# iden3/wasmsnark

Measured on AMD Instinct MI355X. Metric: BN128 Groth16 prove ms @ 2^20 constraints, lower is better.
Workload: dtype u256 (Montgomery; 9x29-bit limbs, v_mad_u64_u32); 1 GPU; BN128 full Groth16 prove, synthetic 2^20-constraint R1CS (1-3 non-zeros per column of A and B, every variable present), key and witness resident in HBM, r and s injected; parallelism=1 GPU, no collective, lanes=2, device=AMD Radeon Graphics gfx950:sramecc+:xnack- CUs=256 device=0

## Files before the change

wasmsnark_amd/csrc/msm.hip:

```cpp
#include <string.h>

#include <algorithm>
#include <chrono>

#include "internal.h"
namespace wsnark {

#ifndef WS_ACC_WAVES
#define WS_ACC_WAVES 3
#endif
#ifndef WS_ACC_WAVES_G2
#define WS_ACC_WAVES_G2 2
#endif
#ifndef WS_G2_PREFETCH
#define WS_G2_PREFETCH 0
#endif
#ifndef WS_G1_PREFETCH
#define WS_G1_PREFETCH 1
#endif
#ifndef WS_MADD_WIDE
#define WS_MADD_WIDE 1
#endif
static const uint32_t CHUNK = 8;
#ifndef WS_TAIL_L2_DEFAULT
#define WS_TAIL_L2_DEFAULT 4
#endif

struct MsmScratch {
    DevBuf vals_out, entries, hot, hot_sums;
    DevBuf bstart, bend, buckets, counters, tasks, multi, partials;
    DevBuf chunkS, chunkA, sums, points_conv;
    DevBuf hot_done;
    DevBuf tree_half, tree_done;
};

static const uint32_t PRESORT_MAX_BINS = 4096;
static const uint32_t CNT_HIST = 16, CNT_CURSOR = 16 + 512, CNT_BINS = 2048;

template <class Fn>
__device__ __forceinline__ void for_each_digit(const Fe& raw, uint32_t c, uint32_t Wall, uint32_t w_off, uint32_t w_stride, Fn f) {
    const Fe s = Fr::reduce_full(raw);
    const uint32_t NB = 1u << (c - 1);
    uint32_t carry = 0, k = 0;
    for (uint32_t w = 0; w < Wall; w++) {
        const uint32_t bit = w * c;
        const uint32_t limb = bit >> 6, off = bit & 63;
        uint64_t v = limb < 4 ? (s.l[limb] >> off) : 0;
        if (off + c > 64 && limb + 1 < 4) v |= s.l[limb + 1] << (64 - off);
        uint32_t d = (uint32_t)(v & ((1u << c) - 1)) + carry;
        uint32_t neg = 0;
        if (d > NB) { d = (1u << c) - d; neg = 1; carry = 1; } else carry = 0;
        if (w >= w_off && (w - w_off) % w_stride == 0) {
            if (d) f(k, d, neg);
            k++;
        }
    }
}

struct PresortArgs {
    const Fe* scalars;
    uint32_t n, c, Wall, w_off, w_stride;
    uint32_t i0, i_end;
    uint32_t lo_bits, HB, nbins;
    uint32_t tile;
    uint32_t idx_bits;
    const uint8_t* mask;
    uint32_t flat;
};
__device__ __forceinline__ uint32_t presort_bin(const PresortArgs& A, uint32_t k, uint32_t d) {
    return (A.flat ? 0u : k * A.HB) + ((d - 1) >> A.lo_bits);
}

template <class E> struct PresortEntry;
template <> struct PresortEntry<uint64_t> {
    static __device__ __forceinline__ uint64_t make(uint32_t i, uint32_t neg, uint32_t lo, uint32_t) {
        return ((uint64_t)lo << 32) | (uint64_t)(i | (neg << 31));
    }
    static __device__ __forceinline__ uint32_t lo(uint64_t e, uint32_t) { return (uint32_t)(e >> 32); }
    static __device__ __forceinline__ uint32_t val(uint64_t e, uint32_t) { return (uint32_t)e; }
};
template <> struct PresortEntry<uint32_t> {
    static __device__ __forceinline__ uint32_t make(uint32_t i, uint32_t neg, uint32_t lo, uint32_t ib) {
        return i | (neg << ib) | (lo << (ib + 1));
    }
    static __device__ __forceinline__ uint32_t lo(uint32_t e, uint32_t ib) { return e >> (ib + 1); }
    static __device__ __forceinline__ uint32_t val(uint32_t e, uint32_t ib) {
        return (e & ((1u << ib) - 1)) | (((e >> ib) & 1u) << 31);
    }
};

// ... 199 lines not shown
    if (act == 0) return 0;
    const uint32_t lane = threadIdx.x & 63;
    const int first = __ffsll(act) - 1;
    const uint32_t k0 = __shfl(key, first);
    const unsigned long long same = __ballot(active && key == k0);
    uint32_t r = 0;
    if (same == act) {
        uint32_t base = 0;
        if (lane == (uint32_t)first) base = atomicAdd(&counters[k0], (uint32_t)__popcll(act));
        base = __shfl(base, first);
        r = base + (uint32_t)__popcll(act & ((1ull << lane) - 1));
    } else if (active) {
        r = atomicAdd(&counters[key], 1u);
    }
    return r;
}

__device__ __forceinline__ uint32_t presort_bins_bounds(uint32_t bin, uint32_t s, uint32_t lo_bits, uint32_t lmax, uint32_t* sub, uint32_t* off,
                                                        uint32_t* wsum, uint32_t* lhist, uint32_t* __restrict__ bstart,
                                                        uint32_t* __restrict__ bend, uint32_t* __restrict__ hist) {
    const uint32_t SUB = 1u << lo_bits;
    const uint32_t per = (SUB + blockDim.x - 1) / blockDim.x, t0 = threadIdx.x * per;
    uint32_t mine = 0, bin_total;
    for (uint32_t t = t0; t < t0 + per && t < SUB; t++) mine += sub[t];
    uint32_t run = s + block_exclusive_scan(mine, wsum, &bin_total);
    for (uint32_t t = t0; t < t0 + per && t < SUB; t++) {
        const uint32_t cnt = sub[t];
        const uint32_t bucket = (bin << lo_bits) + t;
        off[t] = run;
        bstart[bucket] = run;
        bend[bucket] = run + cnt;
        run += cnt;
        sub[t] = 0;
        if (cnt) {
            const uint32_t nt = (cnt + lmax - 1) / lmax, rem = cnt - (nt - 1) * lmax;
            if (nt > 1) atomicAdd(&lhist[255], nt - 1);
            atomicAdd(&lhist[len_key(rem, lmax)], 1u);
        }
    }
    __syncthreads();
    for (uint32_t t = threadIdx.x; t < 256; t += blockDim.x)
        if (lhist[t]) atomicAdd(&hist[t], lhist[t]);
    return bin_total;
}

static const uint32_t PRESORT_BINS_CAP = 4096;
static_assert(PRESORT_BINS_CAP < 0xFFFFu, "ranks are kept in 16 bits, 0xFFFF marks a masked entry");
static_assert(PRESORT_BINS_CAP * (4 + 4 + 2) + (2u << PRESORT_MAX_LO) * 4 + (17 + 256) * 4 <= PRESORT_LDS_BYTES / 3, "staged presort_bins: three workgroups per CU");
template <class E, bool STAGED>
__global__ __launch_bounds__(1024) void presort_bins(const E* __restrict__ entries, const uint32_t* __restrict__ bin_start,
                                                       uint32_t lo_bits, uint32_t idx_bits, uint32_t* __restrict__ vals_out,
                                                       uint32_t* __restrict__ bstart, uint32_t* __restrict__ bend,
                                                       uint32_t lmax, uint32_t* __restrict__ hist,
                                                       const uint8_t* __restrict__ mask, uint32_t mask_mod) {
    __shared__ uint32_t sub[1u << PRESORT_MAX_LO];
    __shared__ uint32_t off[1u << PRESORT_MAX_LO];
    __shared__ uint32_t wsum[17];
    __shared__ uint32_t lhist[256];
    const uint32_t bin = blockIdx.x, SUB = 1u << lo_bits;
    const uint32_t s = bin_start[bin], e = bin_start[bin + 1];
    for (uint32_t t = threadIdx.x; t < SUB; t += blockDim.x) sub[t] = 0;
    for (uint32_t t = threadIdx.x; t < 256; t += blockDim.x) lhist[t] = 0;
    __syncthreads();
    const uint32_t stride = 4 * blockDim.x;
    const uint32_t iters = (e - s + stride - 1) / stride;
    const bool staged = STAGED && e - s <= PRESORT_BINS_CAP;
    (void)staged;
    if constexpr (STAGED) {
        __shared__ uint32_t st_in[PRESORT_BINS_CAP];
        __shared__ uint32_t st_out[PRESORT_BINS_CAP];
        __shared__ uint16_t st_rank[PRESORT_BINS_CAP];
        if (staged) {
            for (uint32_t it = 0; it < iters; it++) {
                const uint32_t i = s + threadIdx.x + it * stride;
                E v[4];
#pragma unroll
                for (uint32_t u = 0; u < 4; u++) {
                    const uint32_t j = i + u * blockDim.x;
                    v[u] = j < e ? entries[j] : (E)0;
                }
#pragma unroll
                for (uint32_t u = 0; u < 4; u++) {
                    const uint32_t j = i + u * blockDim.x;
                    bool active = j < e;
                    if (mask && active) {
                        const uint32_t idx = PresortEntry<E>::val(v[u], idx_bits) & 0x7FFFFFFFu;
                        active = mask[mask_mod ? idx % mask_mod : idx] != 0;
                    }
                    const uint32_t r = wave_rank_add(sub, PresortEntry<E>::lo(v[u], idx_bits), active);
                    if (j < e) {
                        st_in[j - s] = (uint32_t)v[u];
                        st_rank[j - s] = active ? (uint16_t)r : (uint16_t)0xFFFFu;
                    }
                }
            }
            __syncthreads();
            const uint32_t kept = presort_bins_bounds(bin, s, lo_bits, lmax, sub, off, wsum, lhist, bstart, bend, hist);
            for (uint32_t j = threadIdx.x; j < e - s; j += blockDim.x) {
                const uint32_t r = st_rank[j];
                if (r != 0xFFFFu) {
                    const E v = (E)st_in[j];
                    st_out[off[PresortEntry<E>::lo(v, idx_bits)] - s + r] = PresortEntry<E>::val(v, idx_bits);
                }
            }
            __syncthreads();
            for (uint32_t j = threadIdx.x; j < kept; j += blockDim.x) vals_out[s + j] = st_out[j];
            return;
        }
    }
    for (uint32_t it = 0; it < iters; it++) {
        const uint32_t i = s + threadIdx.x + it * stride;
        E v[4];
#pragma unroll
// ... 162 lines not shown
        first[threadIdx.x] += v;
        __syncthreads();
    }
    if (blockIdx.x == 0 && threadIdx.x == 0) counters[3] = first[0];
    const uint32_t excl = threadIdx.x + 1 < 256 ? first[threadIdx.x + 1] : 0;
    __syncthreads();
    first[threadIdx.x] = excl;
    __syncthreads();
    const uint32_t b = blockIdx.x * blockDim.x + threadIdx.x;
    uint32_t cnt = 0, s = 0, nt = 0, rem = 0, krem = 0, r255 = 0, rrem = 0;
    if (b < nbuckets) {
        s = bstart[b];
        cnt = bend[b] - s;
        if (cnt) {
            nt = (cnt + lmax - 1) / lmax;
            rem = cnt - (nt - 1) * lmax;
            krem = len_key(rem, lmax);
            if (nt > 1) r255 = atomicAdd(&lcnt[255], nt - 1);
            rrem = atomicAdd(&lcnt[krem], 1u);
        }
    }
    __syncthreads();
    lbase[threadIdx.x] = lcnt[threadIdx.x] ? first[threadIdx.x] + atomicAdd(&cursor[threadIdx.x], lcnt[threadIdx.x]) : 0;
    __syncthreads();
    if (!cnt) return;
    if (nt == 1) {
        tasks[lbase[krem] + rrem] = Task{b, s, rem};
    } else {
        const uint32_t pbase = atomicAdd(&counters[0], nt);
        if (nt >= hot_min) {
            const uint32_t nsl = (nt + HOT_SLICE - 1) / HOT_SLICE;
            hot[atomicAdd(&counters[4], 1u)] = HotBucket{b, pbase, nt, lbase[255] + r255, lbase[krem] + rrem, s, rem,
                                                         atomicAdd(&counters[5], nsl)};
            return;
        }
        multi[atomicAdd(&counters[1], 1u)] = MultiBucket{b, pbase, nt};
        for (uint32_t k = 0; k + 1 < nt; k++) tasks[lbase[255] + r255 + k] = Task{PARTIAL_FLAG | (pbase + k), s + k * lmax, lmax};
        tasks[lbase[krem] + rrem] = Task{PARTIAL_FLAG | (pbase + nt - 1), s + (nt - 1) * lmax, rem};
    }
}

__global__ __launch_bounds__(256) void msm_plan_emit_hot(const HotBucket* __restrict__ hot, const uint32_t* __restrict__ counters,
                                                           uint32_t lmax, Task* __restrict__ tasks) {
    const uint32_t nhot = counters[4];
    for (uint32_t hb = blockIdx.x; hb < nhot; hb += gridDim.x) {
        const HotBucket h = hot[hb];
        for (uint32_t k = threadIdx.x; k + 1 < h.ntasks; k += blockDim.x)
            tasks[h.task_base + k] = Task{PARTIAL_FLAG | (h.first_partial + k), h.start + k * lmax, lmax};
        if (threadIdx.x == 0)
            tasks[h.rem_index] = Task{PARTIAL_FLAG | (h.first_partial + h.ntasks - 1), h.start + (h.ntasks - 1) * lmax, h.rem};
    }
}

template <class C>
struct AccSets {
    const typename C::AffP* points[4];
    const uint32_t* vals[4];
    const Task* tasks[4];
    const uint32_t* counters[4];
    const MultiBucket* multi[4];
    const HotBucket* hot[4];
    typename C::PtP* buckets[4];
    typename C::PtP* partials[4];
    typename C::PtP* hot_sums[4];
    uint32_t* hot_done[4];
};

template <class C>
__global__ __launch_bounds__(256, (sizeof(typename C::PtP) > 128 ? WS_ACC_WAVES_G2 : WS_ACC_WAVES)) void msm_accumulate(AccSets<C> as) {
    const typename C::AffP* __restrict__ points = as.points[blockIdx.y];
    const uint32_t* __restrict__ vals = as.vals[blockIdx.y];
    const Task* __restrict__ tasks = as.tasks[blockIdx.y];
    const uint32_t* __restrict__ counters = as.counters[blockIdx.y];
    typename C::PtP* __restrict__ buckets = as.buckets[blockIdx.y];
    typename C::PtP* __restrict__ partials = as.partials[blockIdx.y];
    const uint32_t t = blockIdx.x * blockDim.x + threadIdx.x;
    if (t >= counters[3]) return;
    const Task k = tasks[t];
    const typename C::PtP acc = C::pack_pt(accumulate_range<C>(points, vals, k.start, k.len));
    if (k.dst & PARTIAL_FLAG) partials[k.dst & ~PARTIAL_FLAG] = acc;
    else buckets[k.dst] = acc;
}

static const uint32_t WAVE_COMBINE_MIN = 17;
static const uint32_t CB_SMALL_MIN = 256, CB_SMALL_MAX = 4096, CB_WAVE = 256, CB_HOT = 256;
template <class C>
__device__ __forceinline__ typename C::Pt wave_tree_sum(typename C::PtP* sh, uint32_t lane, const typename C::Pt& mine) {
    sh[lane] = C::pack_pt(mine);
    __syncthreads();
    for (uint32_t step = 32; step >= 1; step >>= 1) {
        if (lane < step) sh[lane] = C::pack_pt(C::add(C::unpack_pt(sh[lane]), C::unpack_pt(sh[lane + step])));
        __syncthreads();
    }
    const typename C::Pt r = C::unpack_pt(sh[0]);
    __syncthreads();
    return r;
}
template <class C>
__global__ __launch_bounds__(64) void msm_combine_all(AccSets<C> as, uint32_t CB_SMALL) {
    const uint32_t* __restrict__ counters = as.counters[blockIdx.y];
    const typename C::PtP* __restrict__ partials = as.partials[blockIdx.y];
    typename C::PtP* __restrict__ buckets = as.buckets[blockIdx.y];
    __shared__ typename C::PtP sh[64];
    const uint32_t lane = threadIdx.x;
    if (blockIdx.x < CB_SMALL) {
        const MultiBucket* __restrict__ mbs = as.multi[blockIdx.y];
// ... 299 lines not shown
    int plan_id = 0;
    MsmPlanInfo info;
    DevBuf d_sums, d_rows;
    MsmScratch S;
    void* h_sums = nullptr;
    size_t h_bytes = 0;
    hipEvent_t ev = nullptr;
    hipEvent_t ev_chunks = nullptr;
    const void* d_points_used = nullptr;
    int partner = -1;
    void release() {
        if (h_sums) (void)hipHostFree(h_sums);
        if (ev) (void)hipEventDestroy(ev);
        if (ev_chunks) (void)hipEventDestroy(ev_chunks);
        h_sums = nullptr; ev = ev_chunks = nullptr; h_bytes = 0; active = false;
        d_sums.release(); d_rows.release();
        S.buckets.release(); S.partials.release(); S.chunkS.release(); S.chunkA.release(); S.points_conv.release(); S.hot_sums.release();
        S.hot_done.release(); S.tree_half.release(); S.tree_done.release();
    }
};

static const int kPlans = 4;
static const int kPendingSlots = 8;
struct MsmWorkspace {
    struct Plan { MsmPlanInfo info; MsmScratch S; } plan[kPlans];
    int cur = 0;
    MsmPending slot[kPendingSlots];
    hipEvent_t host_ev = nullptr;
    hipEvent_t conv_ev[2] = {nullptr, nullptr};
    DevBuf conv_buf;
};
static MsmWorkspace& ws(Lane& L) {
    if (!L.msm) L.msm = new MsmWorkspace();
    return *L.msm;
}
void msm_workspace_free(Lane& L) {
    if (!L.msm) return;
    MsmWorkspace& M = *L.msm;
    if (M.host_ev) (void)hipEventDestroy(M.host_ev);
    for (auto& e : M.conv_ev) if (e) (void)hipEventDestroy(e);
    for (auto& p : M.slot) p.release();
    delete L.msm;
    L.msm = nullptr;
}
void msm_select_plan(Lane& L, int id) { ws(L).cur = (id >= 0 && id < kPlans) ? id : 0; }

void msm_abort_slots(Lane& L, const int* slots, int nslots, hipStream_t a, hipStream_t b) {
    if (a) (void)hipStreamSynchronize(a);
    if (b && b != a) (void)hipStreamSynchronize(b);
    if (L.stream3 && L.stream3 != a && L.stream3 != b) (void)hipStreamSynchronize(L.stream3);
    if (!L.msm) return;
    for (int k = 0; k < nslots; k++)
        if (slots[k] >= 0 && slots[k] < kPendingSlots) L.msm->slot[slots[k]].active = false;
}

template <class H, class HPt = typename H::Pt>
static HPt horner_table_folded(const MsmTail& G, const HPt* sums) {
    const uint32_t logm = ceil_log2(G.m), logt = ceil_log2(G.tNB), logP = ceil_log2(G.tP);
    HPt acc = H::infinity();
    for (int q = (int)G.logJ - 1; q >= 0; q--) acc = H::add(H::dbl(acc), sums[q]);
    if (G.m2 > 1) {
        const uint32_t logm1 = ceil_log2(G.m1);
        for (uint32_t k = logm1; k < logm; k++) acc = H::dbl(acc);
        acc = H::add(acc, sums[G.logJ + 1 + logP]);
        for (uint32_t k = 0; k < logm1; k++) acc = H::dbl(acc);
    } else {
        for (uint32_t k = 0; k < logm; k++) acc = H::dbl(acc);
    }
    acc = H::add(acc, sums[G.logJ]);
    HPt tot = H::infinity();
    for (int pb = (int)logP - 1; pb >= 0; pb--) tot = H::add(H::dbl(tot), sums[G.logJ + 1 + (uint32_t)pb]);
    for (uint32_t k = 0; k < logt; k++) tot = H::dbl(tot);
    return H::add(acc, tot);
}
template <class H, class HPt = typename H::Pt>
static HPt horner_table_pieces(const MsmTail& G, const HPt* sums) {
    const uint32_t logm = ceil_log2(G.m), logt = ceil_log2(G.tNB);
    HPt acc = H::infinity();
    for (int q = (int)G.logJ - 1; q >= 0; q--) {
        acc = H::dbl(acc);
        for (uint32_t v = 0; v < G.tW; v++) acc = H::add(acc, sums[(size_t)v * G.nsum + q]);
    }
    for (uint32_t k = 0; k < logm; k++) acc = H::dbl(acc);
    for (uint32_t v = 0; v < G.tW; v++) acc = H::add(acc, sums[(size_t)v * G.nsum + G.logJ]);
    if (G.tW > 1) {
        HPt run = H::infinity(), tot = H::infinity();
        for (uint32_t v = G.tW - 1; v >= 1; v--) {
            run = H::add(run, sums[(size_t)v * G.nsum + G.logJ + 1]);
            tot = H::add(tot, run);
        }
        for (uint32_t k = 0; k < logt; k++) tot = H::dbl(tot);
        acc = H::add(acc, tot);
    }
    return acc;
}
template <class H, class HPt = typename H::Pt>
static HPt horner_windows(const MsmShape& Sh, const MsmTail& G, const HPt* sums) {
    const uint32_t logm = ceil_log2(G.m), logt = ceil_log2(G.tNB), logP = ceil_log2(G.tP);
    const uint32_t rows_per_window = G.reduce ? G.nrows : G.nsum;
    HPt acc = H::infinity();
    bool started = false;
    for (int wg = (int)Sh.Wall - 1; wg >= 0; wg--) {
        const bool owned = (uint32_t)wg >= Sh.w_off && ((uint32_t)wg - Sh.w_off) % Sh.w_stride == 0;
        const uint32_t krow = owned ? ((uint32_t)wg - Sh.w_off) / Sh.w_stride : 0;
        const HPt* row = owned ? &sums[(size_t)krow * rows_per_window] : nullptr;
        for (int k = (int)Sh.c - 1; k >= 0; k--) {
// ... 85 lines not shown
    G.nsum = G.logJ + 1 + ((I.flat || G.tP > 1) ? 1 : 0) + (G.m2 > 1 ? 1 : 0);
    G.reduce = G.tP > 1;
    G.nrows = G.reduce ? G.logJ + 1 + ceil_log2(G.tP) + (G.m2 > 1 ? 1 : 0) : G.nsum;
    I.lmax = (uint32_t)(2 * (((I.flat ? total : n) + I.NB - 1) / I.NB));
    if (I.flat && I.NB < (1u << 19) && total >= ((uint64_t)1 << 22) && total / I.NB > 64) {
        const uint32_t by_tasks = (uint32_t)((total + (1u << 19) - 1) >> 19);
        if (I.lmax > by_tasks) I.lmax = by_tasks;
    }
    uint32_t lmin = 32;
    if (I.nbuckets < (1u << 16) && total >= ((uint64_t)1 << 16)) {
        const uint32_t by_tasks = (uint32_t)((total + (1u << 17) - 1) >> 17);
        if (by_tasks < I.lmax) I.lmax = by_tasks;
        lmin = 8;
    } else if (I.flat && I.nbuckets == (1u << 16) && I.lmax > 16) {
        I.lmax = 16;
        lmin = 16;
    }
    { const long v = tuning_get("MSM_LMAX", 0); if (v >= 4 && v <= 65536) { I.lmax = (uint32_t)v; lmin = 4; } }
    if (I.lmax < lmin) I.lmax = lmin;
    I.hot_cap = (uint32_t)(total / I.lmax) + I.nbuckets + 16;
    { const long v = tuning_get("MSM_HOT_MIN", 0); I.hot_min = v >= 2 ? (uint32_t)v : HOT_MIN; }

    MsmGrouping& ps = info->ps;
    const uint32_t c = I.c;
    uint32_t& lo_bits = ps.lo_bits = 8;
    { const long v = tuning_get("MSM_LO_BITS", 0); if (v >= 1 && v <= (long)PRESORT_MAX_LO) lo_bits = (uint32_t)v; }
    const bool env_e64 = tuning_get("MSM_ENTRY64", 0) != 0;
    if (lo_bits > c - 1) lo_bits = c - 1;
    const uint32_t Wb = I.flat ? 1 : I.W;
    while ((uint64_t)Wb * (I.NB >> lo_bits) > PRESORT_MAX_BINS && lo_bits < c - 1 && lo_bits < PRESORT_MAX_LO) lo_bits++;
    while (I.flat && (I.NB >> lo_bits) < 2048 && lo_bits > 7) lo_bits--;
    const uint32_t idx_bits = ps.idx_bits = std::max(1u, ceil_log2(I.flat ? (uint64_t)I.Wall * n : n));
    while (!env_e64 && idx_bits + 1 + lo_bits > 32 && lo_bits > 1 && (uint64_t)Wb * (I.NB >> (lo_bits - 1)) <= PRESORT_MAX_BINS) lo_bits--;
    ps.HB = I.NB >> lo_bits;
    ps.nbins = Wb * ps.HB;
    if (ps.nbins > PRESORT_MAX_BINS) { set_last_error("msm: grouping pass geometry out of range"); return WS_ERR_SIZE; }
    ps.e32 = !env_e64 && idx_bits + 1 + lo_bits <= 32;
    ps.valid = true;
    return WS_OK;
}

static int reserve_plan_buffers(MsmScratch& S, const MsmPlanInfo& info) {
    const MsmShape& I = info.shape;
    WS_HIP_CHECK(S.vals_out.reserve(I.n * I.W * 4));
    WS_HIP_CHECK(S.bstart.reserve((size_t)I.nbuckets * 4));
    WS_HIP_CHECK(S.bend.reserve((size_t)I.nbuckets * 4));
    WS_HIP_CHECK(S.counters.reserve((size_t)CNT_BINS * 4 + ((size_t)PRESORT_MAX_BINS + 1) * 4 * 3));
    WS_HIP_CHECK(S.tasks.reserve((size_t)I.hot_cap * sizeof(Task)));
    WS_HIP_CHECK(S.multi.reserve((size_t)I.hot_cap * sizeof(MultiBucket)));
    WS_HIP_CHECK(S.hot.reserve(((size_t)I.hot_cap / I.hot_min + 16) * sizeof(HotBucket)));
    return WS_OK;
}

int msm_plan_begin(Lane& L, uint64_t n, WindowShard sh, hipStream_t s, uint32_t table_c) {
    if (!ctx()) return WS_ERR_NOINIT;
    if (!s) s = L.stream;
    MsmWorkspace& M = ws(L);
    MsmPlanInfo& I = M.plan[M.cur].info;
    int rc = msm_plan_geometry(n, sh, table_c, &I);
    if (rc || I.shape.n == 0) return rc;
    if ((rc = wait_plan_users(M, M.cur, s))) return rc;
    MsmScratch& S = M.plan[M.cur].S;
    if ((rc = reserve_plan_buffers(S, I))) return rc;
    WS_HIP_CHECK(S.entries.reserve(I.shape.n * I.shape.W * (I.ps.e32 ? 4 : 8)));
    WS_HIP_CHECK(hipMemsetAsync(S.counters.p, 0, (CNT_BINS + 3 * ((size_t)I.ps.nbins + 1)) * 4, s));
    I.building = true;
    return WS_OK;
}

static bool presort_stage_scatter() { const long v = tuning_get("PRESORT_STAGE", 1); return v == 1 || v == 2; }
static bool presort_stage_bins() { const long v = tuning_get("PRESORT_STAGE", 1); return v == 1 || v == 3; }

static int launch_bins_and_tasks(const MsmPlanInfo& info, const MsmScratch& src, MsmScratch& S, const uint8_t* mask, uint32_t mask_mod, hipStream_t s) {
    KernelTimer& T = ctx()->timer;
    const MsmGrouping& ps = info.ps;
    const uint32_t nbuckets = info.shape.nbuckets, lmax = info.shape.lmax;
    const dim3 grid(ps.nbins), blk(ps.bthr);
    const uint32_t* bin_start = src.counters.as<uint32_t>() + CNT_BINS + (ps.nbins + 1);
    uint32_t* d_cnt = S.counters.as<uint32_t>();
    uint32_t* hist = d_cnt + CNT_HIST;
    uint32_t* vals = S.vals_out.as<uint32_t>();
    uint32_t* bs = S.bstart.as<uint32_t>();
    uint32_t* be = S.bend.as<uint32_t>();
    T.begin("msm_presort_bins", s);
    if (ps.e32 && presort_stage_bins())
        hipLaunchKernelGGL((presort_bins<uint32_t, true>), grid, blk, 0, s, src.entries.as<uint32_t>(), bin_start, ps.lo_bits, ps.idx_bits, vals, bs, be, lmax, hist, mask, mask_mod);
    else if (ps.e32)
        hipLaunchKernelGGL((presort_bins<uint32_t, false>), grid, blk, 0, s, src.entries.as<uint32_t>(), bin_start, ps.lo_bits, ps.idx_bits, vals, bs, be, lmax, hist, mask, mask_mod);
    else
        hipLaunchKernelGGL((presort_bins<uint64_t, false>), grid, blk, 0, s, src.entries.as<uint64_t>(), bin_start, ps.lo_bits, ps.idx_bits, vals, bs, be, lmax, hist, mask, mask_mod);
    T.end(s);
    WS_HIP_CHECK(hipGetLastError());
    T.begin("msm_plan", s);
    hipLaunchKernelGGL(msm_plan_emit, dim3(ceil_div_u64(nbuckets, 256)), dim3(256), 0, s, bs, be, nbuckets, lmax, hist, d_cnt + CNT_CURSOR,
                       S.tasks.as<Task>(), d_cnt, S.multi.as<MultiBucket>(), S.hot.as<HotBucket>(), info.shape.hot_min);
    hipLaunchKernelGGL(msm_plan_emit_hot, dim3(64), dim3(256), 0, s, S.hot.as<HotBucket>(), d_cnt, lmax, S.tasks.as<Task>());
    T.end(s);
    WS_HIP_CHECK(hipGetLastError());
    return WS_OK;
}

static PresortArgs plan_presort_args(const MsmPlanInfo& info, const Fe* d_scalars, uint32_t i0, uint32_t i_end) {
    const MsmShape& I = info.shape;
    const MsmGrouping& ps = info.ps;
    return PresortArgs{d_scalars, (uint32_t)I.n, I.c, I.Wall, I.w_off, I.w_stride, i0, i_end, ps.lo_bits, ps.HB, ps.nbins, ps.tile,
                       ps.idx_bits, nullptr, I.flat ? 1u : 0u};
}

int msm_plan_count(Lane& L, const Fe* d_scalars, uint64_t i0, uint64_t i1, hipStream_t s) {
    Context* X = ctx();
    if (!X) return WS_ERR_NOINIT;
    if (!s) s = L.stream;
    MsmWorkspace& M = ws(L);
    MsmPlanInfo& I = M.plan[M.cur].info;
    if (I.shape.n == 0 && I.valid) return WS_OK;
    if (!I.building) { set_last_error("msm_plan_count: no plan is being built"); return WS_ERR_ARG; }
    if (!d_scalars || i0 > i1 || i1 > I.shape.n) return WS_ERR_ARG;
    if (i0 == i1) return WS_OK;
    MsmScratch& S = M.plan[M.cur].S;
    uint32_t* bin_count = S.counters.as<uint32_t>() + CNT_BINS;
    const PresortArgs PA = plan_presort_args(I, d_scalars, (uint32_t)i0, (uint32_t)i1);
    X->timer.begin("msm_presort_count", s);
    hipLaunchKernelGGL(presort_count, dim3(ceil_div_u64(i1 - i0, I.ps.tile)), dim3(I.ps.thr), 0, s, PA, bin_count);
    X->timer.end(s);
    WS_HIP_CHECK(hipGetLastError());
    return WS_OK;
}

int msm_plan_finish(Lane& L, const Fe* d_scalars, hipStream_t s) {
    Context* X = ctx();
    if (!X) return WS_ERR_NOINIT;
    if (!s) s = L.stream;
    MsmWorkspace& M = ws(L);
    MsmPlanInfo& I = M.plan[M.cur].info;
    if (I.shape.n == 0 && I.valid) return WS_OK;
    if (!I.building) { set_last_error("msm_plan_finish: no plan is being built"); return WS_ERR_ARG; }
    if (!d_scalars) return WS_ERR_ARG;
    I.building = false;
    MsmScratch& S = M.plan[M.cur].S;
    KernelTimer& T = X->timer;
    const uint64_t n = I.shape.n, total = n * I.shape.W;
    const uint32_t nbins = I.ps.nbins;
    const bool e32 = I.ps.e32;
    uint32_t* bin_count = S.counters.as<uint32_t>() + CNT_BINS;
    uint32_t* bin_start = bin_count + (nbins + 1);
    uint32_t* bin_cursor = bin_start + (nbins + 1);
    const PresortArgs PA = plan_presort_args(I, d_scalars, 0u, (uint32_t)n);
    const dim3 grid(ceil_div_u64(n, I.ps.tile)), blk(I.ps.thr);
    const bool once = I.shape.Wall <= PRESORT_ONCE_W && I.ps.tile == I.ps.thr;
    if (!once) {
        T.begin("msm_presort_scan", s);
        hipLaunchKernelGGL(presort_scan, dim3(1), dim3(256), 0, s, bin_count, nbins, bin_start, bin_cursor);
        T.end(s);
    }
    T.begin("msm_presort_scatter", s);
    if (once && e32 && presort_stage_scatter())
        hipLaunchKernelGGL((presort_scatter_once<uint32_t, true>), grid, blk, 0, s, PA, bin_count, bin_start, bin_cursor, S.entries.as<uint32_t>());
    else if (once && e32) hipLaunchKernelGGL((presort_scatter_once<uint32_t, false>), grid, blk, 0, s, PA, bin_count, bin_start, bin_cursor, S.entries.as<uint32_t>());
    else if (once) hipLaunchKernelGGL((presort_scatter_once<uint64_t, false>), grid, blk, 0, s, PA, bin_count, bin_start, bin_cursor, S.entries.as<uint64_t>());
    else if (e32) hipLaunchKernelGGL(presort_scatter<uint32_t>, grid, blk, 0, s, PA, bin_cursor, S.entries.as<uint32_t>());
    else hipLaunchKernelGGL(presort_scatter<uint64_t>, grid, blk, 0, s, PA, bin_cursor, S.entries.as<uint64_t>());
    T.end(s);
    const uint32_t bthr = (uint32_t)((total / nbins / 8 + 63) / 64 * 64);
    I.ps.bthr = bthr < 64 ? 64 : bthr > 1024 ? 1024 : bthr;
    const int rc = launch_bins_and_tasks(I, S, S, nullptr, 0u, s);
    if (rc) return rc;
    I.ntasks = I.shape.hot_cap;
    I.valid = true;
    return WS_OK;
}

int msm_plan_dev(Lane& L, const Fe* d_scalars, uint64_t n, WindowShard sh, hipStream_t s, uint32_t table_c) {
    if (n && !d_scalars) return WS_ERR_ARG;
    int rc = msm_plan_begin(L, n, sh, s, table_c);
    if (!rc) rc = msm_plan_count(L, d_scalars, 0, n, s);
    if (!rc) rc = msm_plan_finish(L, d_scalars, s);
    return rc;
}

int msm_plan_variant(Lane& L, int src_id, int dst_id, const uint8_t* d_mask, hipStream_t s) {
    if (!ctx()) return WS_ERR_NOINIT;
    if (!s) s = L.stream;
    if (src_id < 0 || src_id >= kPlans || dst_id < 0 || dst_id >= kPlans || src_id == dst_id || !d_mask) return WS_ERR_ARG;
    MsmWorkspace& M = ws(L);
    const MsmPlanInfo src = M.plan[src_id].info;
    MsmScratch& SS = M.plan[src_id].S;
    MsmPlanInfo& I = M.plan[dst_id].info;
    MsmScratch& S = M.plan[dst_id].S;
    if (!src.valid || !src.ps.valid || src.shape.n == 0) { set_last_error("msm_plan_variant: the source plan has no shared grouping pass"); return WS_ERR_ARG; }
    int rc = wait_plan_users(M, dst_id, s);
    if (rc) return rc;
    I = src;
    I.ps.valid = false;
    I.valid = false;
    if ((rc = reserve_plan_buffers(S, src))) return rc;
    WS_HIP_CHECK(hipMemsetAsync(S.counters.p, 0, (size_t)CNT_BINS * 4, s));
    if ((rc = launch_bins_and_tasks(src, SS, S, d_mask, src.shape.flat ? (uint32_t)src.shape.n : 0u, s))) return rc;
    I.valid = true;
    return WS_OK;
}

template <class C>
static int msm_acc_sets(Lane& L, MsmPending* const* Ps, int nsets, int which, hipStream_t s) {
    typedef typename C::PtP Pt;
    Context* X = ctx();
    MsmWorkspace& M = ws(L);
    KernelTimer& T = X->timer;
    AccSets<C> as;
    uint32_t ntasks = 0, cb_small = CB_SMALL_MIN;
    for (int k = 0; k < 4; k++) {
        MsmPending& Q = *Ps[k < nsets ? k : 0];
        MsmScratch& QS = M.plan[Q.plan_id].S;
        as.points[k] = reinterpret_cast<const typename C::AffP*>(Q.d_points_used);
        as.vals[k] = QS.vals_out.as<uint32_t>();
        as.tasks[k] = QS.tasks.as<Task>();
        as.counters[k] = QS.counters.as<uint32_t>();
        as.multi[k] = QS.multi.as<MultiBucket>();
        as.hot[k] = QS.hot.as<HotBucket>();
        as.buckets[k] = Q.S.buckets.template as<Pt>();
        as.partials[k] = Q.S.partials.template as<Pt>();
        as.hot_sums[k] = Q.S.hot_sums.template as<Pt>();
        as.hot_done[k] = Q.S.hot_done.template as<uint32_t>();
        if (k < nsets && Q.info.ntasks > ntasks) ntasks = Q.info.ntasks;
        if (k < nsets) {
            const MsmShape& QI = Q.info.shape;
            const uint64_t mean = (QI.n * QI.W + QI.nbuckets - 1) / (QI.nbuckets ? QI.nbuckets : 1);
            if (2 * (uint64_t)QI.lmax < 3 * mean) {
                const uint32_t want = (QI.nbuckets + 63) / 64;
                if (want > cb_small) cb_small = want > CB_SMALL_MAX ? CB_SMALL_MAX : want;
            }
        }
    }
    const uint32_t ny = (uint32_t)nsets;
    T.begin(which ? "msm_accumulate_g2" : "msm_accumulate_g1", s);
    hipLaunchKernelGGL(msm_accumulate<C>, dim3(ceil_div_u64(ntasks, 256), ny), dim3(256), 0, s, as);
    T.end(s);
    WS_HIP_CHECK(hipGetLastError());
    T.begin("msm_combine", s);
    hipLaunchKernelGGL(msm_combine_all<C>, dim3(cb_small + CB_WAVE + CB_HOT, ny), dim3(64), 0, s, as, cb_small);
    T.end(s);
    WS_HIP_CHECK(hipGetLastError());
    return WS_OK;
}

static size_t host_rows_bytes(const MsmPending& P) {
    const MsmTail& G = P.info.tail;
    return (G.reduce ? (size_t)G.groups * G.nrows : (size_t)G.tW * G.nsum) * (P.which ? sizeof(G2::Pt) : sizeof(G1::Pt));
}

template <class C, class H>
static int msm_launch_acc(Lane& L, int which, const typename H::Aff* d_points_ref, bool prepared, int* slot_out, hipStream_t s, bool defer_kernels = false) {
    typedef typename C::PtP Pt;
    static_assert(sizeof(typename C::PtP) == sizeof(typename H::Pt) && sizeof(typename C::AffP) == sizeof(typename H::Aff), "layouts");
    Context* X = ctx();
    if (!X) return WS_ERR_NOINIT;
    if (!s) s = L.stream;
    MsmWorkspace& M = ws(L);
    const MsmPlanInfo& I = M.plan[M.cur].info;
    if (!I.valid) { set_last_error("msm: no plan"); return WS_ERR_ARG; }
    if (I.shape.n && !d_points_ref) return WS_ERR_ARG;
    int slot = -1;
    for (int i = 0; i < kPendingSlots; i++) if (!M.slot[i].active) { slot = i; break; }
    if (slot < 0) { set_last_error("msm: too many unfinished launches"); return WS_ERR_ARG; }
    MsmPending& P = M.slot[slot];
    P.which = which;
    P.info = I;
    P.plan_id = M.cur;
    P.partner = -1;
    if (I.shape.n == 0) { P.active = true; *slot_out = slot; return WS_OK; }
// ... 478 lines not shown
    int rc = msm_dev_t<G2R29, G2>(L, 1, d_scalars, d_points, n, sh, &r, s);
    if (rc) return rc;
    *out_host = G2::to_affine_jac(r);
    return WS_OK;
}
template <class H, class JacT>
static int msm_host_t(Lane& L, int which, const void* h_scalars, const void* h_points, uint64_t n, WindowShard sh, JacT* out_host) {
    if (!ctx()) return WS_ERR_NOINIT;
    if (n == 0) { *out_host = H::to_affine_jac(H::infinity()); return WS_OK; }
    if (!h_scalars || !h_points) return WS_ERR_ARG;
    hipStream_t s = L.stream, s2 = L.stream2;
    MsmWorkspace& M = ws(L);
    WS_HIP_CHECK(L.host_in[0].reserve((size_t)n * 32));
    WS_HIP_CHECK(L.host_in[1].reserve((size_t)n * sizeof(typename H::Aff)));
    if (!M.host_ev) WS_HIP_CHECK(hipEventCreateWithFlags(&M.host_ev, hipEventDisableTiming));
    int rc = upload_staged(L.host_in[0].p, h_scalars, (size_t)n * 32, s);
    if (rc) return rc;
    msm_select_plan(L, 0);
    if ((rc = msm_plan_dev(L, L.host_in[0].as<Fe>(), n, sh, s, 0))) return rc;
    if ((rc = upload_staged(L.host_in[1].p, h_points, (size_t)n * sizeof(typename H::Aff), s2))) return rc;
    WS_HIP_CHECK(hipEventRecord(M.host_ev, s2));
    WS_HIP_CHECK(hipStreamWaitEvent(s, M.host_ev, 0));
    typename H::Pt r;
    int slot = -1;
    rc = which == 0 ? msm_g1_launch(L, reinterpret_cast<const Affine<Fq>*>(L.host_in[1].p), false, &slot, s)
                    : msm_g2_launch(L, reinterpret_cast<const Affine<Fq2>*>(L.host_in[1].p), false, &slot, s);
    if (rc) return rc;
    if ((rc = msm_finish_t<H>(M.slot[slot], &r))) return rc;
    *out_host = H::to_affine_jac(r);
    return WS_OK;
}
int msm_g1_host(Lane& L, const void* h_scalars, const void* h_points, uint64_t n, WindowShard sh, Jac<Fq>* out_host) {
    return msm_host_t<G1, Jac<Fq>>(L, 0, h_scalars, h_points, n, sh, out_host);
}
int msm_g2_host(Lane& L, const void* h_scalars, const void* h_points, uint64_t n, WindowShard sh, Jac<Fq2>* out_host) {
    return msm_host_t<G2, Jac<Fq2>>(L, 1, h_scalars, h_points, n, sh, out_host);
}

int selftest_msm_plan(Lane& L, const void* h_scalars, uint64_t n, uint32_t table_c, WindowShard sh, const uint8_t* h_mask,
                      uint32_t* info, uint32_t* bstart, uint32_t* bend, uint64_t cap_buckets, uint32_t* vals, uint64_t cap_vals,
                      uint32_t* tasks, uint64_t cap_tasks, uint32_t* multi, uint64_t cap_multi, uint32_t* hot, uint64_t cap_hot) {
    static_assert(sizeof(Task) == 12 && sizeof(MultiBucket) == 12 && sizeof(HotBucket) == 32, "record layouts of the hook");
    if (!ctx()) return WS_ERR_NOINIT;
    if (!info || (n && !h_scalars)) return WS_ERR_ARG;
    memset(info, 0, kMsmPlanInfoWords * sizeof(uint32_t));
    hipStream_t s = L.stream;
    MsmWorkspace& M = ws(L);
    int rc;
    if (n) {
        WS_HIP_CHECK(L.host_in[0].reserve((size_t)n * 32));
        if ((rc = upload_staged(L.host_in[0].p, h_scalars, (size_t)n * 32, s))) return rc;
    }
    msm_select_plan(L, 0);
    if ((rc = msm_plan_dev(L, L.host_in[0].as<Fe>(), n, sh, s, table_c))) return rc;
    int id = 0;
    if (h_mask && M.plan[0].info.shape.n) {
        WS_HIP_CHECK(L.host_in[1].reserve((size_t)n));
        if ((rc = upload_staged(L.host_in[1].p, h_mask, (size_t)n, s))) return rc;
        if ((rc = msm_plan_variant(L, 0, 2, L.host_in[1].as<uint8_t>(), s))) return rc;
        id = 2;
    }
    WS_HIP_CHECK(hipStreamSynchronize(s));
    const MsmShape& I = M.plan[id].info.shape;
    const MsmGrouping& ps = M.plan[0].info.ps;
    if (I.n == 0) return WS_OK;
    const MsmScratch& S = M.plan[id].S;
    uint32_t cnt[8], nvals = 0;
    WS_HIP_CHECK(hipMemcpy(cnt, S.counters.p, sizeof cnt, hipMemcpyDeviceToHost));
    WS_HIP_CHECK(hipMemcpy(&nvals, M.plan[0].S.counters.as<uint32_t>() + CNT_BINS + (ps.nbins + 1) + ps.nbins, 4, hipMemcpyDeviceToHost));
    const uint32_t words[kMsmPlanInfoWords] = {
        I.c, I.Wall, I.W, I.w_off, I.w_stride, I.NB, I.nbuckets, I.flat ? 1u : 0u, I.lmax, I.hot_min,
        ps.lo_bits, ps.idx_bits, ps.nbins, ps.e32 ? 1u : 0u, (I.Wall <= PRESORT_ONCE_W && ps.tile == ps.thr) ? 1u : 0u,
        cnt[0], cnt[1], cnt[3], cnt[4], cnt[5], nvals, ps.bthr, (uint32_t)I.n, 0u};
    if (cnt[3] > I.hot_cap || cnt[1] > I.hot_cap || cnt[4] > I.hot_cap / I.hot_min + 16 || (uint64_t)nvals > I.n * I.W) {
        set_last_error("selftest_msm_plan: the plan's counters exceed its buffers");
        return WS_ERR_SIZE;
    }
    if (((bstart || bend) && cap_buckets < I.nbuckets) || (vals && cap_vals < nvals) || (tasks && cap_tasks < cnt[3]) ||
        (multi && cap_multi < cnt[1]) || (hot && cap_hot < cnt[4])) {
        memcpy(info, words, sizeof words);
        set_last_error("selftest_msm_plan: an output array is too small");
        return WS_ERR_SIZE;
    }
    if (bstart) WS_HIP_CHECK(hipMemcpy(bstart, S.bstart.p, (size_t)I.nbuckets * 4, hipMemcpyDeviceToHost));
    if (bend) WS_HIP_CHECK(hipMemcpy(bend, S.bend.p, (size_t)I.nbuckets * 4, hipMemcpyDeviceToHost));
    if (vals && nvals) WS_HIP_CHECK(hipMemcpy(vals, S.vals_out.p, (size_t)nvals * 4, hipMemcpyDeviceToHost));
    if (tasks && cnt[3]) WS_HIP_CHECK(hipMemcpy(tasks, S.tasks.p, (size_t)cnt[3] * sizeof(Task), hipMemcpyDeviceToHost));
    if (multi && cnt[1]) WS_HIP_CHECK(hipMemcpy(multi, S.multi.p, (size_t)cnt[1] * sizeof(MultiBucket), hipMemcpyDeviceToHost));
    if (hot && cnt[4]) WS_HIP_CHECK(hipMemcpy(hot, S.hot.p, (size_t)cnt[4] * sizeof(HotBucket), hipMemcpyDeviceToHost));
    memcpy(info, words, sizeof words);
    return WS_OK;
}

int selftest_msm_geometry(uint64_t n, uint32_t table_c, WindowShard sh, uint32_t* words) {
    memset(words, 0, kMsmGeometryWords * sizeof(uint32_t));
    MsmPlanInfo info;
    const int rc = msm_plan_geometry(n, sh, table_c == kMsmTableAuto ? msm_table_window(n) : table_c, &info);
    const MsmShape& I = info.shape;
    const MsmGrouping& ps = info.ps;
    const MsmTail& G = info.tail;
    if (rc || I.n == 0) return rc;
    const uint32_t w[kMsmGeometryWords] = {
        (uint32_t)I.n, I.c, I.Wall, I.W, I.w_off, I.w_stride, I.NB, I.nbuckets, I.flat ? 1u : 0u, I.lmax, I.hot_min, I.hot_cap,
        ps.lo_bits, ps.idx_bits, ps.nbins, ps.bthr, ps.HB, ps.tile, ps.thr, ps.valid ? 1u : 0u, ps.e32 ? 1u : 0u,
        G.tW, G.tNB, G.tP, G.groups, G.m1, G.m2, G.m, G.J1, G.J, G.logJ, G.nsum, G.nrows, G.reduce};
    memcpy(words, w, sizeof w);
    return WS_OK;
}

static const uint8_t kAccHookFill = 0xA5;
template <class C>
__global__ __launch_bounds__(256) void acc_hook_export(const typename C::PtP* __restrict__ buckets, const typename C::PtP* __restrict__ partials,
                                                         typename C::PtP* __restrict__ out, uint32_t ntasks) {
    const uint32_t t = blockIdx.x * blockDim.x + threadIdx.x;
    if (t >= ntasks) return;
    out[t] = C::pt_from_internal(C::unpack_pt((t & 1) ? partials[t] : buckets[t]));
}
template <class C, class H>
static int selftest_msm_accumulate_t(int which, const void* h_points, uint64_t n_points, const uint32_t* h_vals, uint64_t n_vals,
                                     const uint32_t* h_tasks, uint64_t n_tasks, uint8_t* out, hipStream_t s) {
    typedef typename C::PtP PtP;
    static_assert(sizeof(PtP) == sizeof(typename H::Pt), "layouts");
    const uint32_t nt = (uint32_t)n_tasks;
    const size_t slots = (size_t)nt + 256;
    std::vector<Task> tasks(nt);
    for (uint32_t t = 0; t < nt; t++) tasks[t] = Task{(t & 1) ? (PARTIAL_FLAG | t) : t, h_tasks[2 * t], h_tasks[2 * t + 1]};
// ... 87 lines not shown
```

Before: 8.390 ms.

## Fuse MSM plan emit kernels and skip counter memsets via double-buffered self-clearing counters

Result: faster. 8.250 ms (median of 6 runs) (-1.7%).

```diff
diff --git a/wasmsnark_amd/csrc/msm.hip b/wasmsnark_amd/csrc/msm.hip
--- a/wasmsnark_amd/csrc/msm.hip
+++ b/wasmsnark_amd/csrc/msm.hip
@@ -32,10 +32,16 @@
     DevBuf chunkS, chunkA, sums, points_conv;
     DevBuf hot_done;
     DevBuf tree_half, tree_done;
+    uint32_t blk = 0;
+    bool hdr_clean = false;
+    uint32_t bins_clean = 0;
+    const void* cnt_ptr = nullptr;
+    hipStream_t cnt_stream = nullptr;
+    bool fused = false;
 };
 
 static const uint32_t PRESORT_MAX_BINS = 4096;
-static const uint32_t CNT_HIST = 16, CNT_CURSOR = 16 + 512, CNT_BINS = 2048;
+static const uint32_t CNT_HIST = 16, CNT_CURSOR = 16 + 512, CNT_ARRIVE = 7, CNT_BLOCK = 2048, CNT_BINS = 2 * CNT_BLOCK;
 
 template <class Fn>
 __device__ __forceinline__ void for_each_digit(const Fe& raw, uint32_t c, uint32_t Wall, uint32_t w_off, uint32_t w_stride, Fn f) {
@@ -341,13 +347,14 @@
                                                        uint32_t lo_bits, uint32_t idx_bits, uint32_t* __restrict__ vals_out,
                                                        uint32_t* __restrict__ bstart, uint32_t* __restrict__ bend,
                                                        uint32_t lmax, uint32_t* __restrict__ hist,
-                                                       const uint8_t* __restrict__ mask, uint32_t mask_mod) {
+                                                       const uint8_t* __restrict__ mask, uint32_t mask_mod, uint32_t* __restrict__ bin_dead) {
     __shared__ uint32_t sub[1u << PRESORT_MAX_LO];
     __shared__ uint32_t off[1u << PRESORT_MAX_LO];
     __shared__ uint32_t wsum[17];
     __shared__ uint32_t lhist[256];
     const uint32_t bin = blockIdx.x, SUB = 1u << lo_bits;
     const uint32_t s = bin_start[bin], e = bin_start[bin + 1];
+    if (bin_dead && threadIdx.x == 0) { bin_dead[bin] = 0; bin_dead[2 * (gridDim.x + 1) + bin] = 0; }
     for (uint32_t t = threadIdx.x; t < SUB; t += blockDim.x) sub[t] = 0;
     for (uint32_t t = threadIdx.x; t < 256; t += blockDim.x) lhist[t] = 0;
     __syncthreads();
@@ -616,6 +623,108 @@
     }
 }
 
+static const uint32_t PLAN_THREADS = 512;
+template <uint32_t SPAN>
+__global__ __launch_bounds__(PLAN_THREADS) void msm_plan_fused(const uint32_t* __restrict__ bstart, const uint32_t* __restrict__ bend,
+                                                        uint32_t nbuckets, uint32_t lmax, uint32_t hot_min, uint32_t* counters,
+                                                        Task* tasks, MultiBucket* __restrict__ multi, HotBucket* hot,
+                                                        uint32_t* __restrict__ retired) {
+    constexpr uint32_t THREADS = PLAN_THREADS;
+    static_assert(THREADS % 256 == 0 && THREADS <= 1024 && SPAN % THREADS == 0 && SPAN / THREADS <= 16, "whole rows of buckets, at most 16 per thread; a thread per key");
+    constexpr uint32_t PER = SPAN / THREADS;
+    __shared__ uint32_t lcnt[256];
+    __shared__ uint32_t lbase[256];
+    __shared__ uint32_t first[256];
+    __shared__ uint32_t wsum[17];
+    __shared__ uint32_t wg[5];
+    __shared__ uint32_t wgb[4];
+    const uint32_t tid = threadIdx.x;
+    uint32_t s[PER], cnt[PER];
+#pragma unroll
+    for (uint32_t j = 0; j < PER; j++) {
+        const uint32_t b = blockIdx.x * SPAN + j * THREADS + tid;
+        s[j] = b < nbuckets ? bstart[b] : 0;
+        cnt[j] = b < nbuckets ? bend[b] : 0;
+    }
+    if (blockIdx.x == 0 && retired)
+        for (uint32_t k = tid; k < CNT_BLOCK; k += THREADS) retired[k] = 0;
+    if (tid < 256) lcnt[tid] = 0;
+    if (tid < 5) wg[tid] = 0;
+    {
+        uint32_t total;
+        const uint32_t longer = block_exclusive_scan(tid < 256 ? counters[CNT_HIST + 255 - tid] : 0u, wsum, &total);
+        if (tid < 256) first[255 - tid] = longer;
+        if (blockIdx.x == 0 && tid == 0) counters[3] = total;
+    }
+    __syncthreads();
+    uint32_t r255[PER], rrem[PER], pofs[PER], ridx[PER], hsl[PER];
+#pragma unroll
+    for (uint32_t j = 0; j < PER; j++) {
+        cnt[j] -= s[j];
+        r255[j] = rrem[j] = pofs[j] = ridx[j] = hsl[j] = 0;
+        if (cnt[j]) {
+            const uint32_t nt = (cnt[j] + lmax - 1) / lmax, rem = cnt[j] - (nt - 1) * lmax;
+            if (nt > 1) {
+                r255[j] = atomicAdd(&lcnt[255], nt - 1);
+                pofs[j] = atomicAdd(&wg[0], nt);
+                if (nt >= hot_min) {
+                    ridx[j] = atomicAdd(&wg[2], 1u);
+                    hsl[j] = atomicAdd(&wg[3], (nt + HOT_SLICE - 1) / HOT_SLICE);
+                } else {
+                    ridx[j] = atomicAdd(&wg[1], 1u);
+                }
+            }
+            rrem[j] = atomicAdd(&lcnt[len_key(rem, lmax)], 1u);
+        }
+    }
+    __syncthreads();
+    if (tid < 256) {
+        const uint32_t held = lcnt[tid];
+        lbase[tid] = held ? first[tid] + atomicAdd(&counters[CNT_CURSOR + tid], held) : 0;
+        if (tid < 4) {
+            const uint32_t add = wg[tid];
+            wgb[tid] = add ? atomicAdd(&counters[tid < 2 ? tid : tid + 2], add) : 0;
+        }
+    }
+    __syncthreads();
+    const bool hot_here = wg[2] != 0;
+#pragma unroll
+    for (uint32_t j = 0; j < PER; j++) {
+        if (!cnt[j]) continue;
+        const uint32_t b = blockIdx.x * SPAN + j * THREADS + tid;
+        const uint32_t nt = (cnt[j] + lmax - 1) / lmax, rem = cnt[j] - (nt - 1) * lmax;
+        const uint32_t at_rem = lbase[len_key(rem, lmax)] + rrem[j];
+        if (nt == 1) {
+            tasks[at_rem] = Task{b, s[j], rem};
+            continue;
+        }
+        const uint32_t pbase = wgb[0] + pofs[j], at_full = lbase[255] + r255[j];
+        if (nt >= hot_min) {
+            hot[wgb[2] + ridx[j]] = HotBucket{b, pbase, nt, at_full, at_rem, s[j], rem, wgb[3] + hsl[j]};
+            continue;
+        }
+        multi[wgb[1] + ridx[j]] = MultiBucket{b, pbase, nt};
+        for (uint32_t k = 0; k + 1 < nt; k++) tasks[at_full + k] = Task{PARTIAL_FLAG | (pbase + k), s[j] + k * lmax, lmax};
+        tasks[at_rem] = Task{PARTIAL_FLAG | (pbase + nt - 1), s[j] + (nt - 1) * lmax, rem};
+    }
+    if (hot_here) __threadfence();
+    __syncthreads();
+    if (tid == 0) wg[4] = atomicAdd(&counters[CNT_ARRIVE], 1u) + 1 == gridDim.x ? 1u : 0u;
+    __syncthreads();
+    if (!wg[4]) return;
+    if (tid == 0) counters[CNT_ARRIVE] = 0;
+    const uint32_t nhot = atomicAdd(&counters[4], 0u);
+    if (!nhot) return;
+    __threadfence();
+    for (uint32_t hb = 0; hb < nhot; hb++) {
+        const HotBucket h = hot[hb];
+        for (uint32_t k = tid; k + 1 < h.ntasks; k += THREADS)
+            tasks[h.task_base + k] = Task{PARTIAL_FLAG | (h.first_partial + k), h.start + k * lmax, lmax};
+        if (tid == 0)
+            tasks[h.rem_index] = Task{PARTIAL_FLAG | (h.first_partial + h.ntasks - 1), h.start + (h.ntasks - 1) * lmax, h.rem};
+    }
+}
+
 template <class C>
 struct AccSets {
     const typename C::AffP* points[4];
@@ -1021,6 +1130,7 @@
     if (!L.msm) return;
     for (int k = 0; k < nslots; k++)
         if (slots[k] >= 0 && slots[k] < kPendingSlots) L.msm->slot[slots[k]].active = false;
+    for (auto& p : L.msm->plan) { p.S.hdr_clean = false; p.S.bins_clean = 0; }
 }
 
 template <class H, class HPt = typename H::Pt>
@@ -1212,6 +1322,30 @@
     return WS_OK;
 }
 
+static uint32_t* plan_counters(const MsmScratch& S) { return S.counters.as<uint32_t>() + (size_t)S.blk * CNT_BLOCK; }
+
+static bool plan_fused_switch() { return tuning_get("PLAN_FUSED", 1) != 0; }
+static const uint32_t PLAN_SPAN_DEFAULT = 1024;
+
+static int plan_counters_begin(MsmScratch& S, uint32_t nbins, hipStream_t s) {
+    S.fused = plan_fused_switch();
+    const bool steady = S.fused && S.hdr_clean && S.cnt_ptr == S.counters.p && S.cnt_stream == s && (nbins == 0 || S.bins_clean == nbins);
+    S.hdr_clean = false;
+    if (nbins) S.bins_clean = 0;
+    if (steady) { S.blk ^= 1u; return WS_OK; }
+    S.blk = 0;
+    if (!nbins) S.bins_clean = 0;
+    WS_HIP_CHECK(hipMemsetAsync(S.counters.p, 0, (CNT_BINS + (nbins ? 3 * ((size_t)nbins + 1) : 0)) * 4, s));
+    return WS_OK;
+}
+static void plan_counters_done(MsmScratch& S, uint32_t nbins, hipStream_t s) {
+    if (!S.fused) return;
+    S.hdr_clean = true;
+    if (nbins) S.bins_clean = nbins;
+    S.cnt_ptr = S.counters.p;
+    S.cnt_stream = s;
+}
+
 int msm_plan_begin(Lane& L, uint64_t n, WindowShard sh, hipStream_t s, uint32_t table_c) {
     if (!ctx()) return WS_ERR_NOINIT;
     if (!s) s = L.stream;
@@ -1223,7 +1357,7 @@
     MsmScratch& S = M.plan[M.cur].S;
     if ((rc = reserve_plan_buffers(S, I))) return rc;
     WS_HIP_CHECK(S.entries.reserve(I.shape.n * I.shape.W * (I.ps.e32 ? 4 : 8)));
-    WS_HIP_CHECK(hipMemsetAsync(S.counters.p, 0, (CNT_BINS + 3 * ((size_t)I.ps.nbins + 1)) * 4, s));
+    if ((rc = plan_counters_begin(S, I.ps.nbins, s))) return rc;
     I.building = true;
     return WS_OK;
 }
@@ -1237,24 +1371,37 @@
     const uint32_t nbuckets = info.shape.nbuckets, lmax = info.shape.lmax;
     const dim3 grid(ps.nbins), blk(ps.bthr);
     const uint32_t* bin_start = src.counters.as<uint32_t>() + CNT_BINS + (ps.nbins + 1);
-    uint32_t* d_cnt = S.counters.as<uint32_t>();
+    uint32_t* d_cnt = plan_counters(S);
     uint32_t* hist = d_cnt + CNT_HIST;
+    uint32_t* bin_dead = (S.fused && !mask) ? S.counters.as<uint32_t>() + CNT_BINS : nullptr;
     uint32_t* vals = S.vals_out.as<uint32_t>();
     uint32_t* bs = S.bstart.as<uint32_t>();
     uint32_t* be = S.bend.as<uint32_t>();
     T.begin("msm_presort_bins", s);
     if (ps.e32 && presort_stage_bins())
-        hipLaunchKernelGGL((presort_bins<uint32_t, true>), grid, blk, 0, s, src.entries.as<uint32_t>(), bin_start, ps.lo_bits, ps.idx_bits, vals, bs, be, lmax, hist, mask, mask_mod);
+        hipLaunchKernelGGL((presort_bins<uint32_t, true>), grid, blk, 0, s, src.entries.as<uint32_t>(), bin_start, ps.lo_bits, ps.idx_bits, vals, bs, be, lmax, hist, mask, mask_mod, bin_dead);
     else if (ps.e32)
-        hipLaunchKernelGGL((presort_bins<uint32_t, false>), grid, blk, 0, s, src.entries.as<uint32_t>(), bin_start, ps.lo_bits, ps.idx_bits, vals, bs, be, lmax, hist, mask, mask_mod);
+        hipLaunchKernelGGL((presort_bins<uint32_t, false>), grid, blk, 0, s, src.entries.as<uint32_t>(), bin_start, ps.lo_bits, ps.idx_bits, vals, bs, be, lmax, hist, mask, mask_mod, bin_dead);
     else
-        hipLaunchKernelGGL((presort_bins<uint64_t, false>), grid, blk, 0, s, src.entries.as<uint64_t>(), bin_start, ps.lo_bits, ps.idx_bits, vals, bs, be, lmax, hist, mask, mask_mod);
+        hipLaunchKernelGGL((presort_bins<uint64_t, false>), grid, blk, 0, s, src.entries.as<uint64_t>(), bin_start, ps.lo_bits, ps.idx_bits, vals, bs, be, lmax, hist, mask, mask_mod, bin_dead);
     T.end(s);
     WS_HIP_CHECK(hipGetLastError());
     T.begin("msm_plan", s);
-    hipLaunchKernelGGL(msm_plan_emit, dim3(ceil_div_u64(nbuckets, 256)), dim3(256), 0, s, bs, be, nbuckets, lmax, hist, d_cnt + CNT_CURSOR,
-                       S.tasks.as<Task>(), d_cnt, S.multi.as<MultiBucket>(), S.hot.as<HotBucket>(), info.shape.hot_min);
-    hipLaunchKernelGGL(msm_plan_emit_hot, dim3(64), dim3(256), 0, s, S.hot.as<HotBucket>(), d_cnt, lmax, S.tasks.as<Task>());
+    if (S.fused) {
+        uint32_t* retired = S.counters.as<uint32_t>() + (size_t)(S.blk ^ 1u) * CNT_BLOCK;
+        const long span = tuning_get("PLAN_SPAN", PLAN_SPAN_DEFAULT);
+        auto launch = [&](auto kernel, uint32_t sp) {
+            hipLaunchKernelGGL(kernel, dim3(ceil_div_u64(nbuckets, sp)), dim3(PLAN_THREADS), 0, s, bs, be, nbuckets, lmax, info.shape.hot_min, d_cnt,
+                               S.tasks.as<Task>(), S.multi.as<MultiBucket>(), S.hot.as<HotBucket>(), retired);
+        };
+        if (span == 2048) launch(msm_plan_fused<2048>, 2048u);
+        else if (span == 4096) launch(msm_plan_fused<4096>, 4096u);
+        else launch(msm_plan_fused<PLAN_SPAN_DEFAULT>, PLAN_SPAN_DEFAULT);
+    } else {
+        hipLaunchKernelGGL(msm_plan_emit, dim3(ceil_div_u64(nbuckets, 256)), dim3(256), 0, s, bs, be, nbuckets, lmax, hist, d_cnt + CNT_CURSOR,
+                           S.tasks.as<Task>(), d_cnt, S.multi.as<MultiBucket>(), S.hot.as<HotBucket>(), info.shape.hot_min);
+        hipLaunchKernelGGL(msm_plan_emit_hot, dim3(64), dim3(256), 0, s, S.hot.as<HotBucket>(), d_cnt, lmax, S.tasks.as<Task>());
+    }
     T.end(s);
     WS_HIP_CHECK(hipGetLastError());
     return WS_OK;
@@ -1327,6 +1474,7 @@
     if (rc) return rc;
     I.ntasks = I.shape.hot_cap;
     I.valid = true;
+    plan_counters_done(S, nbins, s);
     return WS_OK;
 }
 
@@ -1354,9 +1502,10 @@
     I.ps.valid = false;
     I.valid = false;
     if ((rc = reserve_plan_buffers(S, src))) return rc;
-    WS_HIP_CHECK(hipMemsetAsync(S.counters.p, 0, (size_t)CNT_BINS * 4, s));
+    if ((rc = plan_counters_begin(S, 0u, s))) return rc;
     if ((rc = launch_bins_and_tasks(src, SS, S, d_mask, src.shape.flat ? (uint32_t)src.shape.n : 0u, s))) return rc;
     I.valid = true;
+    plan_counters_done(S, 0u, s);
     return WS_OK;
 }
 
@@ -1374,7 +1523,7 @@
         as.points[k] = reinterpret_cast<const typename C::AffP*>(Q.d_points_used);
         as.vals[k] = QS.vals_out.as<uint32_t>();
         as.tasks[k] = QS.tasks.as<Task>();
-        as.counters[k] = QS.counters.as<uint32_t>();
+        as.counters[k] = plan_counters(QS);
         as.multi[k] = QS.multi.as<MultiBucket>();
         as.hot[k] = QS.hot.as<HotBucket>();
         as.buckets[k] = Q.S.buckets.template as<Pt>();
@@ -1959,6 +2108,13 @@
         if ((rc = upload_staged(L.host_in[0].p, h_scalars, (size_t)n * 32, s))) return rc;
     }
     msm_select_plan(L, 0);
+    if (n && tuning_get("PLAN_HOOK_ABANDON", 0) != 0) {
+        if ((rc = msm_plan_begin(L, n, sh, s, table_c))) return rc;
+        if ((rc = msm_plan_count(L, L.host_in[0].as<Fe>(), 0, n, s))) return rc;
+        WS_HIP_CHECK(hipStreamSynchronize(s));
+        set_last_error("selftest_msm_plan: the build was abandoned on request (PLAN_HOOK_ABANDON)");
+        return WS_ERR_ARG;
+    }
     if ((rc = msm_plan_dev(L, L.host_in[0].as<Fe>(), n, sh, s, table_c))) return rc;
     int id = 0;
     if (h_mask && M.plan[0].info.shape.n) {
@@ -1973,12 +2129,22 @@
     if (I.n == 0) return WS_OK;
     const MsmScratch& S = M.plan[id].S;
     uint32_t cnt[8], nvals = 0;
-    WS_HIP_CHECK(hipMemcpy(cnt, S.counters.p, sizeof cnt, hipMemcpyDeviceToHost));
+    WS_HIP_CHECK(hipMemcpy(cnt, plan_counters(S), sizeof cnt, hipMemcpyDeviceToHost));
     WS_HIP_CHECK(hipMemcpy(&nvals, M.plan[0].S.counters.as<uint32_t>() + CNT_BINS + (ps.nbins + 1) + ps.nbins, 4, hipMemcpyDeviceToHost));
+    uint32_t left = cnt[CNT_ARRIVE] ? 1u : 0u;
+    {
+        std::vector<uint32_t> w(std::max<size_t>(CNT_BLOCK, 3 * ((size_t)ps.nbins + 1)));
+        WS_HIP_CHECK(hipMemcpy(w.data(), S.counters.as<uint32_t>() + (size_t)(S.blk ^ 1u) * CNT_BLOCK, (size_t)CNT_BLOCK * 4, hipMemcpyDeviceToHost));
+        for (uint32_t k = 0; k < CNT_BLOCK; k++) left += w[k] ? 1u : 0u;
+        if (M.plan[0].S.fused) {
+            WS_HIP_CHECK(hipMemcpy(w.data(), M.plan[0].S.counters.as<uint32_t>() + CNT_BINS, 3 * ((size_t)ps.nbins + 1) * 4, hipMemcpyDeviceToHost));
+            for (uint32_t k = 0; k <= ps.nbins; k++) left += (w[k] ? 1u : 0u) + (w[2 * ((size_t)ps.nbins + 1) + k] ? 1u : 0u);
+        }
+    }
     const uint32_t words[kMsmPlanInfoWords] = {
         I.c, I.Wall, I.W, I.w_off, I.w_stride, I.NB, I.nbuckets, I.flat ? 1u : 0u, I.lmax, I.hot_min,
         ps.lo_bits, ps.idx_bits, ps.nbins, ps.e32 ? 1u : 0u, (I.Wall <= PRESORT_ONCE_W && ps.tile == ps.thr) ? 1u : 0u,
-        cnt[0], cnt[1], cnt[3], cnt[4], cnt[5], nvals, ps.bthr, (uint32_t)I.n, 0u};
+        cnt[0], cnt[1], cnt[3], cnt[4], cnt[5], nvals, ps.bthr, (uint32_t)I.n, left};
     if (cnt[3] > I.hot_cap || cnt[1] > I.hot_cap || cnt[4] > I.hot_cap / I.hot_min + 16 || (uint64_t)nvals > I.n * I.W) {
         set_last_error("selftest_msm_plan: the plan's counters exceed its buffers");
         return WS_ERR_SIZE;
```
